# cgchemlab/chemlab

Measured on AMD Instinct MI355X. Metric: MD steps/sec, 1M-particle reactive LJ melt, higher is better.
Workload: dtype f32; 1 GPU; C5 reactive LJ melt (chain_growth_catalytic shape): 1000000 particles, rho*=0.8, rc=2.5, skin=0.3, dt=0.005, Langevin gamma=5 T=0.5, 4 reactions every 500 steps; melted for 2000 steps before the reactions start; particles=1000000, reaction_interval=500, reaction_events=2189949, parallelism=1 GPU, single domain

## Files before the change

chemlab_amd/csrc/md_kernels.hpp:

```cpp
#pragma once
#include <hip/hip_runtime.h>
#include <stdint.h>

#include "../../include/chem_mi355.h"
#include "../../include/chem_philox.h"
#include "chem_geom_host.hpp"

namespace chem {

template <typename R> struct Vec4T;
template <> struct Vec4T<float> { using type = float4; };
template <> struct Vec4T<double> { using type = double4; };
template <typename R> using Vec4 = typename Vec4T<R>::type;

template <typename R> __device__ __forceinline__ Vec4<R> mk4(R a, R b, R c, R d);
template <> __device__ __forceinline__ float4 mk4<float>(float a, float b, float c, float d) { return make_float4(a, b, c, d); }
template <> __device__ __forceinline__ double4 mk4<double>(double a, double b, double c, double d) { return make_double4(a, b, c, d); }

__device__ __forceinline__ float rint_r(float x) { return rintf(x); }
__device__ __forceinline__ double rint_r(double x) { return rint(x); }
__device__ __forceinline__ float sqrt_r(float x) { return sqrtf(x); }
__device__ __forceinline__ double sqrt_r(double x) { return sqrt(x); }
__device__ __forceinline__ float floor_r(float x) { return floorf(x); }
__device__ __forceinline__ float rcp_r(float x) { return __builtin_amdgcn_rcpf(x); }
// ... 1034 lines not shown
  __syncthreads();
}

template <typename R>
__global__ __launch_bounds__(128) void k_tile_desc(int ntiles, int CAP, const int* __restrict__ cell_start, Box<R> box,
                                                   TileLDS<R>* __restrict__ desc, DevCtl* ctl, const int* __restrict__ cell_sub) {
  if (!ctl->need_rebuild) return;
  __shared__ TileLDS<R> T;
  for (int tile = blockIdx.x; tile < ntiles; tile += gridDim.x) {
    __syncthreads();
    tile_tables<R>(T, CAP, tile, cell_start, box, ctl, cell_sub);
    const int* src = reinterpret_cast<const int*>(&T);
    int* dst = reinterpret_cast<int*>(&desc[tile]);
    for (int k = threadIdx.x; k < (int)(sizeof(TileLDS<R>) / 4); k += blockDim.x) dst[k] = src[k];
  }
}

template <typename R>
__device__ __forceinline__ void tile_load_desc(TileLDS<R>& T, const TileLDS<R>* __restrict__ desc, int tile) {
  const int* src = reinterpret_cast<const int*>(&desc[tile]);
  int* dst = reinterpret_cast<int*>(&T);
  for (int k = threadIdx.x; k < (int)(sizeof(TileLDS<R>) / 4); k += blockDim.x) dst[k] = src[k];
}

template <typename R> __device__ __forceinline__ unsigned char* d3_types(Vec4<R>* sx, int CAP) { return reinterpret_cast<unsigned char*>(sx) + (size_t)(CAP + 1) * 24; }
template <typename R, bool D3>
__device__ __forceinline__ void slot_store(Vec4<R>* const sx, const int CAP, int dst, const Vec4<R>& p) {
  if constexpr (D3) {
    R* s3 = reinterpret_cast<R*>(sx) + 3 * dst;
    s3[0] = p.x; s3[1] = p.y; s3[2] = p.z;
    d3_types<R>(sx, CAP)[dst] = (unsigned char)(int)p.w;
  } else sx[dst] = p;
}
template <typename R, int BS, bool LEAN = false, bool D3 = false, bool QW = false>
__device__ __forceinline__ void tile_fill(const TileLDS<R>& T, Vec4<R>* const sx, const int CAP,
                                          const Vec4<R>* __restrict__ x4, int wmode, const int* __restrict__ tagv = nullptr,
                                          const R* __restrict__ qtag = nullptr, R* const sq = nullptr) {
  constexpr int NW = BS / 64, RPW = (NROW + NW - 1) / NW;
  const int t = threadIdx.x;
  const int w = t >> 6, l = t & 63;
  if (t == 0) slot_store<R, D3>(sx, CAP, T.geom[3], mk4<R>((R)1e18, (R)1e18, (R)1e18, (R)0));
  if constexpr (QW) { if (t == 0) sq[T.geom[3]] = (R)0; }
  if constexpr (LEAN) {
    for (int r = w; r < NROW; r += NW) {
      const int len = T.celloff[r][SX], o0 = T.rowoff[r];
      for (int e = l; e < len; e += 64) {
        int k = 0;
#pragma unroll
        for (int q = 1; q < SX; ++q) k += (e >= T.celloff[r][q]) ? 1 : 0;
        const int g = T.cellg[r][k] + (e - T.celloff[r][k]);
        const int dst = o0 + e;
        if (dst < CAP) {
          Vec4<R> p = x4[g];
          p.x = pos_local(p.x, T.cellshx[r][k], T.org[0], T.qs[0]); p.y = pos_local(p.y, T.rowshy[r], T.org[1], T.qs[1]); p.z = pos_local(p.z, T.rowshz[r], T.org[2], T.qs[2]);
          if (wmode) p.w = idx_as_real((g << 5) | (int)p.w, (R)0);
          slot_store<R, D3>(sx, CAP, dst, p);
        }
      }
    }
    return;
  }
  Vec4<R> pv[RPW][2];
  int pk_[RPW][2], pg[RPW][2];
  [[maybe_unused]] int ptg[RPW][2];
  [[maybe_unused]] R pq[RPW][2];
#pragma unroll
  for (int rr = 0; rr < RPW; ++rr) {
    const int r = w + rr * NW;
    const int len = r < NROW ? T.celloff[r][SX] : 0;
#pragma unroll
    for (int c = 0; c < 2; ++c) {
      const int e = l + 64 * c;
      pk_[rr][c] = -1;
      if (e < len) {
        int k = 0;
#pragma unroll
        for (int q = 1; q < SX; ++q) k += (e >= T.celloff[r][q]) ? 1 : 0;
        const int g = T.cellg[r][k] + (e - T.celloff[r][k]);
        pk_[rr][c] = k; pg[rr][c] = g;
        pv[rr][c] = x4[g];
        if constexpr (QW) ptg[rr][c] = tagv[g];
      }
    }
  }
  if constexpr (QW) {
#pragma unroll
    for (int rr = 0; rr < RPW; ++rr)
#pragma unroll
      for (int c = 0; c < 2; ++c) pq[rr][c] = pk_[rr][c] >= 0 ? qtag[ptg[rr][c]] : (R)0;
  }
#pragma unroll
  for (int rr = 0; rr < RPW; ++rr) {
    const int r = w + rr * NW;
#pragma unroll
    for (int c = 0; c < 2; ++c) {
      const int k = pk_[rr][c];
      if (k >= 0) {
        const int dst = T.rowoff[r] + l + 64 * c;
        if (dst < CAP) {
          Vec4<R> p = pv[rr][c];
          p.x = pos_local(p.x, T.cellshx[r][k], T.org[0], T.qs[0]); p.y = pos_local(p.y, T.rowshy[r], T.org[1], T.qs[1]); p.z = pos_local(p.z, T.rowshz[r], T.org[2], T.qs[2]);
          if (wmode) p.w = idx_as_real((pg[rr][c] << 5) | (int)p.w, (R)0);
          slot_store<R, D3>(sx, CAP, dst, p);
          if constexpr (QW) sq[dst] = pq[rr][c];
        }
      }
    }
  }
  for (int r = w; r < NROW; r += NW) {
    const int len = T.celloff[r][SX], o0 = T.rowoff[r];
    for (int e = l + 128; e < len; e += 64) {
      int k = 0;
#pragma unroll
      for (int q = 1; q < SX; ++q) k += (e >= T.celloff[r][q]) ? 1 : 0;
      const int g = T.cellg[r][k] + (e - T.celloff[r][k]);
      const int dst = o0 + e;
      if (dst < CAP) {
        Vec4<R> p = x4[g];
        p.x = pos_local(p.x, T.cellshx[r][k], T.org[0], T.qs[0]); p.y = pos_local(p.y, T.rowshy[r], T.org[1], T.qs[1]); p.z = pos_local(p.z, T.rowshz[r], T.org[2], T.qs[2]);
        if (wmode) p.w = idx_as_real((g << 5) | (int)p.w, (R)0);
        slot_store<R, D3>(sx, CAP, dst, p);
        if constexpr (QW) sq[dst] = qtag[tagv[g]];
      }
    }
  }
}

struct ActMask { unsigned int row[kMaxTypes]; };
#define CHEM_LDS __attribute__((address_space(3)))
constexpr int NBND = SX * NSUB + 1;
#ifndef CHEM_LIST_DELTA
#define CHEM_LIST_DELTA 2.5e-4f
#endif
constexpr float kListDelta = CHEM_LIST_DELTA;
constexpr int kGrpF = 20;
struct ListLDS { int img_bytes, nwords, tmask_off, bnd_off; };
__device__ __forceinline__ ListLDS list_lds_layout(int CAP, int ntypes) {
  ListLDS L;
  L.img_bytes = (((CAP + 3) >> 2) + 3) * kGrpF * 4;
  L.nwords = ((CAP + 31) >> 5) + 2;
  L.tmask_off = L.img_bytes;
  L.bnd_off = L.tmask_off + ntypes * L.nwords * 4;
  return L;
}
__host__ __device__ constexpr size_t list_lds_bytes(int CAP, int ntypes) {
  return (size_t)(((CAP + 3) >> 2) + 3) * kGrpF * 4 + (size_t)ntypes * (((CAP + 31) >> 5) + 2) * 4 + (size_t)NROW * NBND * 2 + 16;
}

template <int BS>
__device__ __forceinline__ void list_stage_clear(unsigned char* lds, const ListLDS& L, int ntypes) {
  CHEM_LDS unsigned int* tm = (CHEM_LDS unsigned int*)((CHEM_LDS unsigned char*)lds + L.tmask_off);
  for (int k = threadIdx.x; k < ntypes * L.nwords; k += BS) tm[k] = 0u;
}
template <typename RS, int BS>
__device__ __forceinline__ void list_stage_f32(TileLDS<RS>& T, unsigned char* lds, const ListLDS& L, const int CAP,
                                               const Vec4<RS>* __restrict__ x4, const ActMask& act, int ntypes) {
  constexpr int NW = BS / 64;
  CHEM_LDS unsigned char* const l3 = (CHEM_LDS unsigned char*)lds;
  CHEM_LDS float* img = (CHEM_LDS float*)l3;
  CHEM_LDS unsigned int* tm = (CHEM_LDS unsigned int*)(l3 + L.tmask_off);
  CHEM_LDS unsigned short* bnd = (CHEM_LDS unsigned short*)(l3 + L.bnd_off);
  const int w = threadIdx.x >> 6, l = threadIdx.x & 63;
  for (int t = threadIdx.x; t < NROW * NBND; t += BS) {
    const int r = t / NBND, f = t - r * NBND, k = f >> 2, j = f & 3;
    int v = T.celloff[r][k < SX ? k : SX];
    if (k < SX && j) {
      const int pk = T.cellsub[r][k];
      if (pk < 0) { if (T.celloff[r][k + 1] > T.celloff[r][k]) T.geom[7] = 1; }
      else v += (pk >> (8 * (j - 1))) & 0xff;
    }
    bnd[t] = (unsigned short)v;
  }
  for (int r = w; r < NROW; r += NW) {
    const int len = T.celloff[r][SX], o0 = T.rowoff[r];
    for (int e0 = 0; e0 < len; e0 += 64) {
      const int e = e0 + l;
      int tj = -1;
      if (e < len) {
        int k = 0;
#pragma unroll
        for (int q = 1; q < SX; ++q) k += (e >= T.celloff[r][q]) ? 1 : 0;
        const int g = T.cellg[r][k] + (e - T.celloff[r][k]);
        const int dst = o0 + e;
        if (dst < CAP) {
          const Vec4<RS> p = x4[g];
          CHEM_LDS float* grp = img + (dst >> 2) * kGrpF + (dst & 3);
          const float u = (float)pos_local(p.x, T.cellshx[r][k], T.org[0], T.qs[0]), v = (float)pos_local(p.y, T.rowshy[r], T.org[1], T.qs[1]),
                      w_ = (float)pos_local(p.z, T.rowshz[r], T.org[2], T.qs[2]);
          grp[0] = u; grp[4] = v; grp[8] = w_; grp[12] = fmaf(u, u, fmaf(v, v, w_ * w_));
          tj = (int)p.w & 15;
        }
      }
      const int slot0 = o0 + e0, sh = slot0 & 31, wbase = slot0 >> 5;
      for (int ti = 0; ti < ntypes; ++ti) {
        const unsigned long long m = __ballot(tj >= 0 && ((act.row[ti] >> tj) & 1u));
        if (m == 0ull) continue;
        const unsigned long long lo = m << sh;
        const unsigned int w2 = sh ? (unsigned int)(m >> (64 - sh)) : 0u;
        const unsigned int part = l == 0 ? (unsigned int)lo : (l == 1 ? (unsigned int)(lo >> 32) : w2);
        if (l < 3 && part) __hip_atomic_fetch_or(&tm[ti * L.nwords + wbase + l], __brev(part), __ATOMIC_RELAXED, __HIP_MEMORY_SCOPE_WORKGROUP);
      }
    }
  }
}

typedef unsigned int u32x4_t __attribute__((ext_vector_type(4)));
__device__ __forceinline__ uint4 nt_load_u4(const uint4* p) {
  const u32x4_t v = __builtin_nontemporal_load(reinterpret_cast<const u32x4_t*>(p));
  return make_uint4(v.x, v.y, v.z, v.w);
}

__device__ __forceinline__ int xcd_remap(int bid, int nwg) {
  const int q = nwg >> 3, r = nwg & 7, xcd = bid & 7, idx = bid >> 3;
  return (xcd < r ? xcd * (q + 1) : r * (q + 1) + (xcd - r) * q) + idx;
}



template <typename R, int BS>
__device__ __forceinline__ void dev_nlist_tile(const TileLDS<R>& T, Vec4<R>* const sx, const int* tag, const R rl2,
                                               const int* excl_start, const int* excl_list, const int has_excl, const ActMask& act,
                                               unsigned short* nl16, const int S16, int* nnh, int* nlist, const int S, int* nn, DevCtl* ctl,
                                               const Box<R>* bx = nullptr, const int* rtag = nullptr, const Vec4<R>* x4 = nullptr, const R rl2_rows_ = (R)-1) {
    const R rl2_rows = rl2_rows_ > (R)0 ? rl2_rows_ : rl2;
    const int hx = T.geom[0], total = T.geom[3], nhome = T.geom[4], hbase = T.geom[5];
    unsigned short* reg16 = nl16 + (size_t)hbase * S16;
    for (int q = threadIdx.x; q < nhome; q += BS) {
      int sgi = 0;
#pragma unroll
      for (int k = 1; k < NHSEG; ++k) sgi += (q >= T.hoff[k]) ? 1 : 0;
      const int inrun = q - T.hoff[sgi];
      const int p = T.hstart[sgi] + inrun;
      const int ly = sgi % HY, lz = sgi / HY;
      const int hr = (lz + 1) * SY + (ly + 1);
      const int eh = inrun + T.celloff[hr][1];
      int lx = 0;
      for (int k = 2; k <= hx; ++k) lx += (eh >= T.celloff[hr][k]) ? 1 : 0;
      const int sself = T.rowoff[hr] + eh;
      const Vec4<R> xi = sx[sself];
      const unsigned int arow = act.row[real_as_idx(xi.w) & 15];
      int e0 = 0, e1 = 0;
      if (has_excl) { const int tg = tag[p]; e0 = excl_start[tg]; e1 = excl_start[tg + 1]; }
      int cnt = 0, cnt16 = 0;
      int* row32 = nlist ? nlist + (size_t)p * S : nullptr;
      uint4* regq = reinterpret_cast<uint4*>(reg16) + q;
      uint4 acc = make_uint4(0, 0, 0, 0);
      auto push = [&](unsigned int sl) {
        acc.x = __builtin_amdgcn_alignbit(acc.y, acc.x, 16);
        acc.y = __builtin_amdgcn_alignbit(acc.z, acc.y, 16);
        acc.z = __builtin_amdgcn_alignbit(acc.w, acc.z, 16);
        acc.w = (acc.w >> 16) | (sl << 16);
        if ((cnt16 & 7) == 7 && cnt16 < S16) regq[(size_t)(cnt16 >> 3) * nhome] = acc;
        ++cnt16;
      };
      auto hit = [&](int s, int jw) {
        const int j = jw >> 5;
        bool ok = j != p;
        if (ok && e1 > e0) {
          const int tgj = tag[j];
          for (int e = e0; e < e1; ++e) if (excl_list[e] == tgj) { ok = false; break; }
        }
        if (ok) {
          if ((arow >> (jw & 15)) & 1u) push((unsigned int)s);
          if (row32) {
            bool in_rows = true;
            if (rl2_rows < rl2) { const Vec4<R> xj = sx[s]; const R dx = xi.x - xj.x, dy_ = xi.y - xj.y, dz_ = xi.z - xj.z; in_rows = dx * dx + dy_ * dy_ + dz_ * dz_ <= rl2_rows; }
            if (in_rows) { if (cnt < S) row32[cnt] = j; ++cnt; }
          }
        }
      };
      auto suboff = [&](int r, int f, bool lower) {
        const int k = f >> 2, j = f & 3;
        const int base = T.celloff[r][k];
        if (j == 0) return base;
        const int pk = T.cellsub[r][k];
        if (pk < 0) return lower ? base : T.celloff[r][k + 1];
        return base + ((pk >> (8 * (j - 1))) & 0xff);
      };
#pragma unroll 1
      for (int dzy = 0; dzy < 9; ++dzy) {
        const int dz = dzy / 3, dy = dzy - 3 * dz;
        const int r = (lz + dz) * SY + (ly + dy);
        const R weps = T.clen[0] * (R)2e-4;
        const R ylo = ((R)(ly + 1) - (R)kRefCells) * T.clen[1], zlo = ((R)(lz + 1) - (R)kRefCells) * T.clen[2];
        R ddy = dy == 0 ? xi.y - ylo - weps : (dy == 2 ? ylo + T.clen[1] - xi.y - weps : (R)0);
        R ddz = dz == 0 ? xi.z - zlo - weps : (dz == 2 ? zlo + T.clen[2] - xi.z - weps : (R)0);
        ddy = ddy > 0 ? ddy : (R)0; ddz = ddz > 0 ? ddz : (R)0;
        const R w2 = rl2 - ddy * ddy - ddz * ddz;
        if (w2 < (R)0) continue;
        const R ws = (sqrt_r(w2) + weps) * T.subinv, sxi = (xi.x + (R)kRefCells * T.clen[0]) * T.subinv;
        int f_lo = (int)(sxi - ws), f_hi = (int)(sxi + ws);
        f_lo = f_lo > lx * NSUB ? f_lo : lx * NSUB;
        f_hi = f_hi < (lx + 3) * NSUB - 1 ? f_hi : (lx + 3) * NSUB - 1;
        const int a = T.rowoff[r] + suboff(r, f_lo, true);
        int b = T.rowoff[r] + suboff(r, f_hi + 1, false);
        b = b < total ? b : total;
        for (int s0 = a; s0 < b; s0 += 64) {
          const int len = (b - s0) < 64 ? (b - s0) : 64;
          unsigned int mlo = 0, mhi = 0;
          for (int k = 0; k < len; k += 4) {
            Vec4<R> xj[4];
#pragma unroll
            for (int u = 0; u < 4; ++u) xj[u] = sx[(k + u < len) ? s0 + k + u : total];
            unsigned int bits = 0;
#pragma unroll
            for (int u = 0; u < 4; ++u) {
              const R dx = xi.x - xj[u].x, dy_ = xi.y - xj[u].y, dz_ = xi.z - xj[u].z;
              const R r2 = dx * dx + dy_ * dy_ + dz_ * dz_;
              bits |= (r2 <= rl2) ? (1u << u) : 0u;
            }
            if (k < 32) mlo |= bits << k; else mhi |= bits << (k - 32);
          }
          unsigned long long m = ((unsigned long long)mhi << 32) | mlo;
          while (m) {
            const int k = __ffsll((long long)m) - 1;
            m &= m - 1;
            const int s = s0 + k;
            hit(s, real_as_idx(sx[s].w));
          }
        }
      }
      const int real16 = cnt16;
      if (real16 <= S16) while (cnt16 & 7) push((unsigned int)total);
      nnh[hbase + q] = real16 < S16 ? real16 : S16;
      if (real16 > S16) atomicMax(&ctl->nl_overflow, real16);
      if (row32) {
        const int c32 = cnt < S ? cnt : S;
        for (int k = c32; k < ((c32 + 3) & ~3); ++k) row32[k] = p;
        nn[p] = c32;
        if (cnt > S) atomicMax(&ctl->nl_overflow, cnt);
      }
    }
}

template <typename RS, int BS>
__device__ __forceinline__ void dev_nlist_tile_f32(const TileLDS<RS>& T, unsigned char* lds, const ListLDS& L, const int* tag, const float rl2,
                                                   const int* excl_start, const int* excl_list, const int has_excl,
                                                   unsigned short* nl16, const int S16, int* nnh, int* nlist, const int S, int* nn, DevCtl* ctl,
                                                   const Box<RS>* bx, const int* rtag, const Vec4<RS>* x4, const int ablate = 0, const float rl2_rows_ = -1.f,
                                                   uint4* bslots = nullptr, const int* gtag = nullptr, const int real0 = 0, const int real1 = 0x7fffffff,
                                                   const int coop_on = 0) {
  const float rl2_rows = rl2_rows_ > 0.f ? rl2_rows_ : rl2;
  typedef float f32x4 __attribute__((ext_vector_type(4)));
  typedef float f32x2 __attribute__((ext_vector_type(2)));
  typedef __attribute__((address_space(3))) const volatile f32x4 lds_f32x4;
  CHEM_LDS unsigned char* const l3 = (CHEM_LDS unsigned char*)lds;
  const CHEM_LDS float* img = (const CHEM_LDS float*)l3;
  const CHEM_LDS unsigned int* tmask = (const CHEM_LDS unsigned int*)(l3 + L.tmask_off);
  const CHEM_LDS unsigned short* bnd = (const CHEM_LDS unsigned short*)(l3 + L.bnd_off);
  const int hx = T.geom[0], total = T.geom[3], nhome = T.geom[4], hbase = T.geom[5];
  const bool nowin = T.geom[7] != 0;
  unsigned short* reg16 = nl16 + (size_t)hbase * S16;
  const float clen0 = (float)T.clen[0], clen1 = (float)T.clen[1], clen2 = (float)T.clen[2], subinv = (float)T.subinv;
// ... 1042 lines not shown
};

__device__ __forceinline__ bool grid_barrier(GridBar* gb, DevCtl* ctl) {
  __shared__ int ok_s;
  asm volatile("s_waitcnt vmcnt(0)" ::: "memory");
  __syncthreads();
  if (threadIdx.x == 0) {
    __builtin_amdgcn_fence(__ATOMIC_RELEASE, "agent");
    int ok = 1;
    const unsigned int g = blockIdx.x & 7u;
    const unsigned int ngrp = gridDim.x < 8u ? gridDim.x : 8u;
    const unsigned int gsize = (gridDim.x - g + 7u) >> 3;
    const unsigned int gen = __hip_atomic_load(&gb->gen[0], __ATOMIC_RELAXED, __HIP_MEMORY_SCOPE_AGENT);
    if (atomicAdd(&gb->grp[g][0], 1u) == gsize - 1u) {
      __hip_atomic_store(&gb->grp[g][0], 0u, __ATOMIC_RELAXED, __HIP_MEMORY_SCOPE_AGENT);
      if (atomicAdd(&gb->top[0], 1u) == ngrp - 1u) {
        __hip_atomic_store(&gb->top[0], 0u, __ATOMIC_RELAXED, __HIP_MEMORY_SCOPE_AGENT);
        __hip_atomic_fetch_add(&gb->gen[0], 1u, __ATOMIC_RELEASE, __HIP_MEMORY_SCOPE_AGENT);
      }
    }
    unsigned int spins = 0;
    while (__hip_atomic_load(&gb->gen[0], __ATOMIC_RELAXED, __HIP_MEMORY_SCOPE_AGENT) == gen) {
      __builtin_amdgcn_s_sleep(8);
      if (++spins > (1u << 20)) { ctl->barrier_timeout = 1; ok = 0; break; }
    }
    __builtin_amdgcn_fence(__ATOMIC_ACQUIRE, "agent");
    ok_s = ok;
  }
  __syncthreads();
  return ok_s != 0;
}

template <typename R> struct FusedArgs {
  int n, ncell, ntiles, CAP, S, has_excl, criterion, par, seg_shift, tseg_shift, nblk, want32, ntypes, ablate, coop;
  double half_skin; R rl2;
  long long istep;
  double half_skin_ref; R rl2_rows;
  Vec4<R> *x4, *v4, *x4o, *v4o, *x0;
  int *tag, *tago, *rtag; int4 *img4, *img4o;
  int *cell_cnt, *cell_of, *slot_of, *cell_start, *cell_loc, *btot, *perm, *tn, *tloc, *tbtot, *cell_sub, *cell_n, *bucket; int bcap;
  TileLDS<R>* desc; const int *excl_start, *excl_list;
  int* tile_ord;
  int* tile_pos;
  unsigned short* nl16; int *nnh, *nlist, *nn;
  unsigned long long* blockmax; DevCtl* ctl; GridBar* gb;
  const int* bstart; const BondedEntry* bent; int4 *bwork, *bj; int nbent;
  uint4* bslots;
  int bond_pass;
  Box<R> box; ActMask act;
  long long* wgst;
};

template <int BS>
__device__ __forceinline__ void seg_offsets(const int* tot, int nseg, int* s_off) {
  int carry = 0;
  for (int base = 0; base < nseg; base += BS) {
    const int k = base + (int)threadIdx.x;
    const int v = k < nseg ? tot[k] : 0;
    int t;
    const int ex = block_scan_excl<BS>(v, &t);
    if (k < nseg) s_off[k] = carry + ex;
    carry += t;
  }
  if (threadIdx.x == 0) s_off[nseg] = carry;
  __syncthreads();
}

template <int BS>
__device__ __forceinline__ void seg_scan(int* cnt, int nitem, int shift, int* loc, int* tot, bool zero, int* cnt_copy = nullptr) {
  const int per = 1 << shift, nseg = (nitem + per - 1) >> shift;
  for (int seg = blockIdx.x; seg < nseg; seg += gridDim.x) {
    const int lo = seg << shift, hi = min(nitem, lo + per);
    int carry = 0;
    for (int base = lo; base < hi; base += BS) {
      const int k = base + (int)threadIdx.x;
      int v = 0;
      if (k < hi) { v = cnt[k]; if (zero) cnt[k] = 0; if (cnt_copy) cnt_copy[k] = v; }
      int t;
      const int ex = block_scan_excl<BS>(v, &t);
      if (k < hi) loc[k] = carry + ex;
      carry += t;
    }
    if (threadIdx.x == 0) tot[seg] = carry;
  }
}

#ifndef CHEM_FUSED_WAVES
#define CHEM_FUSED_WAVES 4
#endif
template <typename R, int BS, bool DIAG = false>
__global__ __launch_bounds__(BS, CHEM_FUSED_WAVES) void k_rebuild_fused(const FusedArgs<R> a) {
  __shared__ TileLDS<R> T;
  __shared__ int s_off[1025];
  __shared__ unsigned long long s_m[BS / 64];
  __shared__ int s_tile;
  CHEM_DYN_LDS(R);
  const int t = threadIdx.x, b = blockIdx.x, NB = gridDim.x, lane = lane_id(), w = t >> 6;
  DevCtl* const ctl = a.ctl;

  if (ctl->halt) return;
  unsigned long long m = 0;
  for (int k = t; k < a.nblk; k += BS) { const unsigned long long v = a.blockmax[k]; m = v > m ? v : m; }
  for (int o = 32; o > 0; o >>= 1) { const unsigned long long v = __shfl_xor(m, o); m = v > m ? v : m; }
  if (lane == 0) s_m[w] = m;
  __syncthreads();
  m = s_m[0];
#pragma unroll
  for (int k = 1; k < BS / 64; ++k) m = s_m[k] > m ? s_m[k] : m;
  const double m2 = sizeof(R) == 4 ? bits_real_f(m) : bits_real_d(m);
  double acc = a.criterion ? sqrt(m2) : ctl->acc_pp[a.par] + sqrt(m2);
  const int forced = ctl->force_rebuild;
  const int need = (acc > a.half_skin) || forced;
  auto ref_update = [&]() {
    const double accr = a.criterion ? sqrt(m2) : ctl->acc_ref + sqrt(m2);
    const bool rn = (accr > a.half_skin_ref) || forced;
    ctl->acc_ref = rn ? 0.0 : accr;
    if (rn) ctl->ref_rebuilds++;
  };
  if (!need) {
    if (b == 0 && t == 0) { ctl->step_m2 = m2; ctl->acc_pp[a.par ^ 1] = acc; ctl->acc_maxdist = acc; ctl->need_rebuild = 0; ref_update(); }
    return;
  }

  if (b == 0 && t == 0) a.gb->stamp[0] = wall_clock64();
  long long* const wst = (DIAG && a.wgst) ? a.wgst + 8 * (size_t)b : nullptr;
  const int ablate = DIAG ? a.ablate : 0;
#define WGST(K) do { if (wst && t == 0) wst[K] = wall_clock64(); } while (0)
  WGST(0);
  if (b == 0 && t < 8) a.gb->tq[t][0] = 0u;
  if (b == 0 && t == 8) { ctl->bw64 = 0ull; a.gb->prepq[0] = 0u; }
  { MigBuf<R> none{}; dev_bin<R>(0, a.n, a.x4, a.v4, a.tag, a.img4, a.box, a.cell_cnt, a.cell_of, a.slot_of, none, none, ctl, a.bucket, a.bcap, a.btot, a.seg_shift); }
  WGST(1);
  if (!grid_barrier(a.gb, ctl)) return; WGST(2); if (b == 0 && t == 0) { const long long st = wall_clock64(); a.gb->stamp[1] = st; a.gb->stamp[2] = st; a.gb->stamp[3] = st; }
  if (ctl->bucket_overflow) {
    for (int k = b * BS + t; k < a.ncell; k += NB * BS) a.cell_cnt[k] = 0;
    if (b == 0) for (int k = t; k < 1024; k += BS) a.btot[k] = 0;
    if (b == 0 && t == 0) { ctl->need_rebuild = 1; ctl->force_rebuild = 1; ctl->halt_step = a.istep; ctl->halt = 1; }
    return;
  }
  if (b == 0 && t == 0) {
    ctl->step_m2 = m2; ctl->acc_pp[a.par ^ 1] = 0.0; ctl->acc_maxdist = 0.0; ctl->force_rebuild = 0;
    ctl->rebuild_count++; ctl->need_rebuild = 1;
    ref_update();
  }

  {
    const int nseg = (a.ncell + (1 << a.seg_shift) - 1) >> a.seg_shift;
    seg_offsets<BS>(a.btot, nseg, s_off);
    if (b == 0 && t == 0) a.cell_start[a.ncell] = s_off[nseg];
    dev_sort_gather_bucket<R>(a.ncell, a.cell_cnt, s_off, a.seg_shift, a.bucket, a.bcap, a.cell_start, a.x4, a.v4, a.tag, a.img4,
                              a.x4o, a.v4o, a.tago, a.img4o, a.rtag, a.box, a.cell_sub);
    const int nx = a.box.nc[0], ny = a.box.nc[1], nz = a.box.nc[2];
    const int ntx = tile_ntx(nx, a.box.xs_nb, a.box.xs_w), nty = (ny + HY - 1) / HY;
    for (int tile = b * BS + t; tile < a.ntiles; tile += NB * BS) {
      const int tx = tile % ntx, ty = (tile / ntx) % nty, tz = tile / (ntx * nty);
      int cx0, hx;
      tile_xrange(tx, nx, a.box.xs_nb, a.box.xs_w, cx0, hx);
      const int cy0 = ty * HY, cz0 = tz * HZ;
      const int hy = min(HY, ny - cy0), hz = min(HZ, nz - cz0);
      int nh = 0;
      for (int hzi = 0; hzi < hz; ++hzi) for (int hyi = 0; hyi < hy; ++hyi) {
        const int c0 = ((cz0 + hzi) * ny + (cy0 + hyi)) * nx + cx0;
        for (int k = 0; k < hx; ++k) nh += a.cell_cnt[c0 + k];
      }
      a.tn[tile] = nh;
    }
  }
  WGST(3);
  if (!grid_barrier(a.gb, ctl)) return; WGST(4); if (b == 0 && t == 0) { const long long st = wall_clock64(); a.gb->stamp[4] = st; a.gb->stamp[5] = st; }

  {
    for (int k = b * BS + t; k < a.ncell; k += NB * BS) a.cell_cnt[k] = 0;
    if (b == 0) for (int k = t; k < 1024; k += BS) a.btot[k] = 0;
    const int tper = 1 << a.tseg_shift, ntseg = (a.ntiles + tper - 1) >> a.tseg_shift;
    {
      int carry = 0;
      for (int base = 0; base < ntseg; base += BS) {
        const int k = base + t;
        int v = 0;
        if (k < ntseg) for (int j = k << a.tseg_shift; j < min(a.ntiles, (k + 1) << a.tseg_shift); ++j) v += a.tn[j];
        int tot;
        const int ex = block_scan_excl<BS>(v, &tot);
        if (k < ntseg) s_off[k] = carry + ex;
        carry += tot;
      }
      __syncthreads();
    }
    const int q = a.ntiles >> 3, r = a.ntiles & 7, myx = b & 7;
    const int lpar = a.tile_ord ? (ctl->rebuild_count & 1) : 0;
    const int* const ord_r = a.tile_ord ? a.tile_ord + (size_t)lpar * a.ntiles : nullptr;
    const int* const pos_r = a.tile_pos ? a.tile_pos + (size_t)lpar * a.ntiles : nullptr;
    int ndone = 0;
    WGST(5);
    auto claim = [&]() {
      int tile = -1;
      for (int d = 0; d < 8 && tile < 0; ++d) {
        const int x = (myx + d) & 7;
        const int cntx = q + (x < r ? 1 : 0);
        if (__hip_atomic_load(&a.gb->tq[x][0], __ATOMIC_RELAXED, __HIP_MEMORY_SCOPE_AGENT) >= (unsigned int)cntx) continue;
        const int k = (int)atomicAdd(&a.gb->tq[x][0], 1u);
        if (k < cntx) { tile = (x < r ? x * (q + 1) : r * (q + 1) + (x - r) * q) + k; if (ord_r) tile = ord_r[tile]; }
      }
      return tile;
    };
    for (;;) {
      __syncthreads();
      if (t == 0) s_tile = claim();
      __syncthreads();
      const int tile = s_tile;
      if (tile < 0) break;
      ++ndone;
      int hb_part = 0;
      if (w == BS / 64 - 1) {
        for (int j = ((tile >> a.tseg_shift) << a.tseg_shift) + lane; j < tile; j += 64) hb_part += a.tn[j];
      }
      const bool f32list = sizeof(R) == 4 || !(DIAG && a.want32);
      if (f32list) list_stage_clear<BS>(chem_dyn_lds, list_lds_layout(a.CAP, a.ntypes), a.ntypes);
      tile_tables<R>(T, a.CAP, tile, a.cell_start, a.box, ctl, a.cell_sub);
      if (w == BS / 64 - 1) {
        for (int o = 32; o > 0; o >>= 1) hb_part += __shfl_xor(hb_part, o);
        if (lane == 0) T.geom[5] = s_off[tile >> a.tseg_shift] + hb_part;
      }
      __syncthreads();
      {
        const int* src = reinterpret_cast<const int*>(&T);
        int* dst = reinterpret_cast<int*>(&a.desc[pos_r ? pos_r[tile] : tile]);
        for (int k = t; k < (int)(sizeof(TileLDS<R>) / 4); k += BS) dst[k] = src[k];
      }
      if (f32list) {
        const ListLDS L = list_lds_layout(a.CAP, a.ntypes);
        list_stage_f32<R, BS>(T, chem_dyn_lds, L, a.CAP, a.x4o, a.act, a.ntypes);
        __syncthreads();
        if (ablate == 1) { for (int q = t; q < T.geom[4]; q += BS) a.nnh[T.geom[5] + q] = 0; }
        else
        dev_nlist_tile_f32<R, BS>(T, chem_dyn_lds, L, a.tago, (float)a.rl2, a.excl_start, a.excl_list, a.bond_pass ? 0 : a.has_excl, a.nl16, a.S, a.nnh,
                               (DIAG && a.want32) ? a.nlist : (int*)nullptr, a.S, a.nn, ctl, &a.box, a.rtag, a.x4o, ablate, (float)a.rl2_rows,
                               a.bond_pass ? (uint4*)nullptr : a.bslots, nullptr, 0, 0x7fffffff, a.coop);
      } else {
        tile_fill<R, BS, true>(T, sx, a.CAP, a.x4o, 1);
        __syncthreads();
        dev_nlist_tile<R, BS>(T, sx, a.tago, a.rl2, a.excl_start, a.excl_list, a.has_excl, a.act, a.nl16, a.S, a.nnh,
                              a.want32 ? a.nlist : (int*)nullptr, a.S, a.nn, ctl, &a.box, a.rtag, a.x4o, a.rl2_rows);
      }
    }
    WGST(6);
    if (wst && t == 0) wst[7] = ndone;
    if (a.tile_ord && b < 8 && w == 0) {
      const int cntx = q + (b < r ? 1 : 0), off = b < r ? b * (q + 1) : r * (q + 1) + (b - r) * q;
      int* const ord_w = a.tile_ord + (size_t)(lpar ^ 1) * a.ntiles;
      int* const pos_w = a.tile_pos + (size_t)(lpar ^ 1) * a.ntiles;
      const int mean4 = (int)(((long long)a.n * 4 + a.ntiles - 1) / a.ntiles);
      auto cls_of = [&](int tile) { const int c = a.tn[tile] * 16 / (mean4 > 0 ? mean4 : 1); return 7 - (c > 7 ? 7 : c); };
      int tot[8] = {0, 0, 0, 0, 0, 0, 0, 0};
      for (int k0 = 0; k0 < cntx; k0 += 64) {
        const int k = k0 + lane, c = k < cntx ? cls_of(off + k) : -1;
#pragma unroll
        for (int cc = 0; cc < 8; ++cc) tot[cc] += __popcll(__ballot(c == cc));
      }
      int base[8]; { int acc_ = 0;
#pragma unroll
        for (int cc = 0; cc < 8; ++cc) { base[cc] = acc_; acc_ += tot[cc]; } }
      for (int k0 = 0; k0 < cntx; k0 += 64) {
        const int k = k0 + lane, c = k < cntx ? cls_of(off + k) : -1;
#pragma unroll
        for (int cc = 0; cc < 8; ++cc) {
          const unsigned long long m = __ballot(c == cc);
          if (c == cc) { const int p_ = off + base[cc] + __popcll(m & lanemask_lt()); ord_w[p_] = off + k; pos_w[off + k] = p_; }
          base[cc] += __popcll(m);
        }
      }
    }
    if (a.nbent > 0) {
      for (;;) {
        __syncthreads();
        if (t == 0) s_tile = (int)atomicAdd(&a.gb->prepq[0], 1u);
        __syncthreads();
        const int ib = s_tile * BS;
        if (ib >= a.n) break;
        dev_bonded_prep_chunk<BS>(ib, a.n, a.tago, a.rtag, a.bstart, a.bent, a.bwork, a.bj, ctl, a.bslots ? a.excl_start : (const int*)nullptr);
      }
    }
    for (int k = b * BS + t; k < a.n; k += NB * BS) {
      const Vec4<R> xk = a.x4o[k];
      a.x4[k] = xk; if (a.x0) a.x0[k] = xk;
      a.v4[k] = a.v4o[k]; a.img4[k] = a.img4o[k]; a.tag[k] = a.tago[k];
    }
  }
  if (t == 0) {
    const volatile DevCtl* vc = ctl;
    if (vc->stage_overflow | vc->nl_overflow) { ctl->halt_step = a.istep; ctl->halt = 1; }
  }
  if (b == 0 && t == 0) a.gb->stamp[6] = wall_clock64();
  if (wst) { __syncthreads(); if (t == 0) wst[7] |= (long long)(wall_clock64() - wst[0]) << 16; }
#undef WGST
}

template <typename R>
__global__ __launch_bounds__(256) void k_kinetic(int i0, int n, const Vec4<R>* __restrict__ v4, double* __restrict__ out) {
  const int i = i0 + blockIdx.x * blockDim.x + threadIdx.x;
  double ek = 0, px = 0, py = 0, pz = 0;
  if (i < i0 + n) {
    const Vec4<R> v = v4[i];
    const double m = (double)v.w, vx = (double)v.x, vy = (double)v.y, vz = (double)v.z;
    ek = 0.5 * m * (vx * vx + vy * vy + vz * vz); px = m * vx; py = m * vy; pz = m * vz;
  }
  __shared__ double red[4][4];
  for (int o = 32; o > 0; o >>= 1) { ek += __shfl_xor(ek, o); px += __shfl_xor(px, o); py += __shfl_xor(py, o); pz += __shfl_xor(pz, o); }
  if (lane_id() == 0) { int w = threadIdx.x >> 6; red[0][w] = ek; red[1][w] = px; red[2][w] = py; red[3][w] = pz; }
  __syncthreads();
  if (threadIdx.x < 4) {
    double s = 0;
    for (int k = 0; k < (int)(blockDim.x >> 6); ++k) s += red[threadIdx.x][k];
    out[4 * blockIdx.x + threadIdx.x] = s;
  }
}

__global__ __launch_bounds__(256) void k_rescale_lambda(const double* __restrict__ part, int nblk, double* __restrict__ ekin_io, double* __restrict__ lam_out,
                                                        int kind, double kT, double pref , double ntot, uint64_t svr_seed, uint64_t step) {
  __shared__ double red[4];
  double ek = 0;
  for (int k = threadIdx.x; k < nblk; k += blockDim.x) ek += part[4 * k];
  for (int o = 32; o > 0; o >>= 1) ek += __shfl_xor(ek, o);
  if (lane_id() == 0) red[threadIdx.x >> 6] = ek;
  __syncthreads();
  if (threadIdx.x == 0) {
    if (nblk > 0) { ek = red[0] + red[1] + red[2] + red[3]; *ekin_io = ek; }
    else ek = *ekin_io;
    if (lam_out) {
      const double kTnow = 2.0 * ek / (3.0 * ntot);
      *lam_out = kind == 1 ? sqrt(1.0 + pref * (kT / kTnow - 1.0)) : kind == 2 ? sqrt(kT / kTnow)
               : chem_philox::svr_lambda(svr_seed, step, ek, 1.5 * ntot * kT, (int64_t)(3.0 * ntot), 1.0 / pref);
    }
  }
}
template <typename R>
__global__ __launch_bounds__(256) void k_scale_v(int i0, int n, Vec4<R>* __restrict__ v4, const double* __restrict__ lam, const DevCtl* __restrict__ ctl) {
  if (ctl->halt) return;
  const int i = i0 + blockIdx.x * blockDim.x + threadIdx.x;
  if (i >= i0 + n) return;
  const R s = (R)*lam;
  Vec4<R> v = v4[i];
  v.x *= s; v.y *= s; v.z *= s;
  v4[i] = v;
}

struct ReactionDev {
  int type_1, type_2, delta_1, delta_2;
  int min1, max1, min2, max2;
  int intramolecular, intraresidual, active, restricted;
  int cons_role, pad_;
  double cut2, mincut2, prob;
};
struct ReactSet { int n; uint64_t seed; uint64_t step; int nearest; ReactionDev r[CHEM_MAX_REACTIONS]; };
struct ConnTable { const int* start; const int* partner; const unsigned int* mask; const unsigned int* cons_ok; };
__device__ __forceinline__ bool conn_allows(const ConnTable& ct, int ta, int tb, int q) {
  if (!ct.start) return false;
  for (int e = ct.start[ta]; e < ct.start[ta + 1]; ++e) if (ct.partner[e] == tb) return (ct.mask[e] >> q) & 1u;
  return false;
}

struct Candidate { int a, b, r; unsigned int h; double d2; };

template <typename R>
__global__ __launch_bounds__(256) void k_react_scan(int i0, int n, const Vec4<R>* __restrict__ x4, const int* __restrict__ tag,
                                                    const int* __restrict__ nlist, const int* __restrict__ nn, int S,
                                                    const int* __restrict__ state, const int* __restrict__ res_id,
                                                    const int* __restrict__ mol_id, BoxD box, const ReactSet* __restrict__ rs_g,
                                                    Candidate* __restrict__ cand, int cand_cap, DevCtl* ctl, ConnTable conn) {
  __shared__ ReactSet rs;
  {
    const int* src = reinterpret_cast<const int*>(rs_g);
    int* dst = reinterpret_cast<int*>(&rs);
    for (int k = threadIdx.x; k < (int)(sizeof(ReactSet) / 4); k += blockDim.x) dst[k] = src[k];
  }
  __syncthreads();
  constexpr int TPP = 8;
  constexpr int kWaveBuf = 192;
  __shared__ Candidate sbuf[4 * kWaveBuf];
  Candidate* wbuf = sbuf + (threadIdx.x >> 6) * kWaveBuf;
  int wcount = 0;
  const int gid = blockIdx.x * blockDim.x + threadIdx.x;
  const int i = i0 + gid / TPP, sub = gid % TPP;
  int cnt = 0, ti = 0, si = 0, tgi = 0, ri = 0, mi = 0;
  Vec4<R> xi = mk4<R>(0, 0, 0, 0);
  const int* row = nullptr;
  if (i < i0 + n) {
    xi = x4[i]; ti = (int)xi.w; tgi = tag[i]; si = state[tgi]; ri = res_id[tgi]; mi = mol_id[tgi];
    cnt = nn[i]; row = nlist + (size_t)i * S;
    bool any = false;
    for (int q = 0; q < rs.n; ++q) {
      const ReactionDev& R_ = rs.r[q];
// ... 590 lines not shown
```

Baseline: 7430 steps/s.

## Restructure neighbor-list staging as flat slot sweep with prefetched loads overlapping descriptor write

The per-tile list staging now walks all slots of the tile flatly across the whole block instead of per-row per-wave. It issues up to NF position loads per thread into registers before doing the descriptor finish, barrier and bound-table work, so global latency overlaps that setup. Because each wave now covers 32-aligned slots, the type-mask atomics become plain stores. Per-tile home counts are also computed one wave per tile with one lane per cell and a shuffle reduction, instead of one thread looping serially. The trade-offs are more register pressure from the prefetch arrays and a geom[7] flag that is now written as zero into the global descriptor.

```diff
diff --git a/chemlab_amd/csrc/md_kernels.hpp b/chemlab_amd/csrc/md_kernels.hpp
--- a/chemlab_amd/csrc/md_kernels.hpp
+++ b/chemlab_amd/csrc/md_kernels.hpp
@@ -1210,53 +1210,75 @@
   CHEM_LDS unsigned int* tm = (CHEM_LDS unsigned int*)((CHEM_LDS unsigned char*)lds + L.tmask_off);
   for (int k = threadIdx.x; k < ntypes * L.nwords; k += BS) tm[k] = 0u;
 }
-template <typename RS, int BS>
+struct StageNoMid { __device__ __forceinline__ void operator()() const {} };
+template <typename RS, int BS, typename Mid = StageNoMid>
 __device__ __forceinline__ void list_stage_f32(TileLDS<RS>& T, unsigned char* lds, const ListLDS& L, const int CAP,
-                                               const Vec4<RS>* __restrict__ x4, const ActMask& act, int ntypes) {
-  constexpr int NW = BS / 64;
+                                               const Vec4<RS>* __restrict__ x4, const ActMask& act, int ntypes, Mid&& mid = Mid()) {
+  static_assert(BS % 64 == 0 && NROW <= 64, "a wave stages 64 consecutive slots; one lane per row offset");
+  constexpr int NF = sizeof(RS) == 8 ? 3 : 6;
   CHEM_LDS unsigned char* const l3 = (CHEM_LDS unsigned char*)lds;
   CHEM_LDS float* img = (CHEM_LDS float*)l3;
   CHEM_LDS unsigned int* tm = (CHEM_LDS unsigned int*)(l3 + L.tmask_off);
   CHEM_LDS unsigned short* bnd = (CHEM_LDS unsigned short*)(l3 + L.bnd_off);
-  const int w = threadIdx.x >> 6, l = threadIdx.x & 63;
-  for (int t = threadIdx.x; t < NROW * NBND; t += BS) {
-    const int r = t / NBND, f = t - r * NBND, k = f >> 2, j = f & 3;
-    int v = T.celloff[r][k < SX ? k : SX];
-    if (k < SX && j) {
-      const int pk = T.cellsub[r][k];
-      if (pk < 0) { if (T.celloff[r][k + 1] > T.celloff[r][k]) T.geom[7] = 1; }
-      else v += (pk >> (8 * (j - 1))) & 0xff;
-    }
-    bnd[t] = (unsigned short)v;
-  }
-  for (int r = w; r < NROW; r += NW) {
-    const int len = T.celloff[r][SX], o0 = T.rowoff[r];
-    for (int e0 = 0; e0 < len; e0 += 64) {
-      const int e = e0 + l;
-      int tj = -1;
-      if (e < len) {
+  const int l = threadIdx.x & 63;
+  const int total = T.rowoff[NROW], lim = total < CAP ? total : CAP;
+  const int ro_l = T.rowoff[l < NROW ? l : NROW];
+  int ro[NROW];
+#pragma unroll
+  for (int q = 1; q < NROW; ++q) ro[q] = __builtin_amdgcn_readlane(ro_l, q);
+  for (int s0 = 0; s0 < lim; s0 += NF * BS) {
+    Vec4<RS> pv[NF];
+    int prk[NF];
+#pragma unroll
+    for (int c = 0; c < NF; ++c) {
+      const int s = s0 + c * BS + (int)threadIdx.x;
+      prk[c] = -1;
+      if (s < lim) {
+        int r = 0, o0 = 0;
+#pragma unroll
+        for (int q = 1; q < NROW; ++q) if (s >= ro[q]) { r = q; o0 = ro[q]; }
+        const int e = s - o0;
         int k = 0;
 #pragma unroll
         for (int q = 1; q < SX; ++q) k += (e >= T.celloff[r][q]) ? 1 : 0;
         const int g = T.cellg[r][k] + (e - T.celloff[r][k]);
-        const int dst = o0 + e;
-        if (dst < CAP) {
-          const Vec4<RS> p = x4[g];
-          CHEM_LDS float* grp = img + (dst >> 2) * kGrpF + (dst & 3);
-          const float u = (float)pos_local(p.x, T.cellshx[r][k], T.org[0], T.qs[0]), v = (float)pos_local(p.y, T.rowshy[r], T.org[1], T.qs[1]),
-                      w_ = (float)pos_local(p.z, T.rowshz[r], T.org[2], T.qs[2]);
-          grp[0] = u; grp[4] = v; grp[8] = w_; grp[12] = fmaf(u, u, fmaf(v, v, w_ * w_));
-          tj = (int)p.w & 15;
+        prk[c] = (r << 3) | k;
+        pv[c] = x4[g];
+      }
+    }
+    if (s0 == 0) {
+      mid();
+      for (int t = threadIdx.x; t < NROW * NBND; t += BS) {
+        const int r = t / NBND, f = t - r * NBND, k = f >> 2, j = f & 3;
+        int v = T.celloff[r][k < SX ? k : SX];
+        if (k < SX && j) {
+          const int pk = T.cellsub[r][k];
+          if (pk < 0) { if (T.celloff[r][k + 1] > T.celloff[r][k]) T.geom[7] = 1; }
+          else v += (pk >> (8 * (j - 1))) & 0xff;
         }
-      }
-      const int slot0 = o0 + e0, sh = slot0 & 31, wbase = slot0 >> 5;
+        bnd[t] = (unsigned short)v;
+      }
+    }
+#pragma unroll
+    for (int c = 0; c < NF; ++c) {
+      const int slot0 = s0 + c * BS + ((int)threadIdx.x & ~63);
+      if (slot0 >= lim) continue;
+      int tj = -1;
+      if (prk[c] >= 0) {
+        const int r = prk[c] >> 3, k = prk[c] & 7, dst = slot0 + l;
+        const Vec4<RS> p = pv[c];
+        CHEM_LDS float* grp = img + (dst >> 2) * kGrpF + (dst & 3);
+        const float u = (float)pos_local(p.x, T.cellshx[r][k], T.org[0], T.qs[0]), v = (float)pos_local(p.y, T.rowshy[r], T.org[1], T.qs[1]),
+                    w_ = (float)pos_local(p.z, T.rowshz[r], T.org[2], T.qs[2]);
+        grp[0] = u; grp[4] = v; grp[8] = w_; grp[12] = fmaf(u, u, fmaf(v, v, w_ * w_));
+        tj = (int)p.w & 15;
+      }
+      const int wbase = slot0 >> 5;
       for (int ti = 0; ti < ntypes; ++ti) {
         const unsigned long long m = __ballot(tj >= 0 && ((act.row[ti] >> tj) & 1u));
         if (m == 0ull) continue;
-        const unsigned long long lo = m << sh;
-        const unsigned int w2 = sh ? (unsigned int)(m >> (64 - sh)) : 0u;
-        const unsigned int part = l == 0 ? (unsigned int)lo : (l == 1 ? (unsigned int)(lo >> 32) : w2);
-        if (l < 3 && part) __hip_atomic_fetch_or(&tm[ti * L.nwords + wbase + l], __brev(part), __ATOMIC_RELAXED, __HIP_MEMORY_SCOPE_WORKGROUP);
+        const unsigned int part = l == 0 ? (unsigned int)m : (unsigned int)(m >> 32);
+        if (l < 2 && part) tm[ti * L.nwords + wbase + l] = __brev(part);
       }
     }
   }
@@ -2605,18 +2627,17 @@
                               a.x4o, a.v4o, a.tago, a.img4o, a.rtag, a.box, a.cell_sub);
     const int nx = a.box.nc[0], ny = a.box.nc[1], nz = a.box.nc[2];
     const int ntx = tile_ntx(nx, a.box.xs_nb, a.box.xs_w), nty = (ny + HY - 1) / HY;
-    for (int tile = b * BS + t; tile < a.ntiles; tile += NB * BS) {
+    static_assert(HX * HY * HZ <= 64, "one lane per home cell");
+    for (int tile = b * (BS / 64) + w; tile < a.ntiles; tile += NB * (BS / 64)) {
       const int tx = tile % ntx, ty = (tile / ntx) % nty, tz = tile / (ntx * nty);
       int cx0, hx;
       tile_xrange(tx, nx, a.box.xs_nb, a.box.xs_w, cx0, hx);
       const int cy0 = ty * HY, cz0 = tz * HZ;
       const int hy = min(HY, ny - cy0), hz = min(HZ, nz - cz0);
-      int nh = 0;
-      for (int hzi = 0; hzi < hz; ++hzi) for (int hyi = 0; hyi < hy; ++hyi) {
-        const int c0 = ((cz0 + hzi) * ny + (cy0 + hyi)) * nx + cx0;
-        for (int k = 0; k < hx; ++k) nh += a.cell_cnt[c0 + k];
-      }
-      a.tn[tile] = nh;
+      const int k = lane % HX, hyi = (lane / HX) % HY, hzi = lane / (HX * HY);
+      int nh = (k < hx && hyi < hy && hzi < hz) ? a.cell_cnt[((cz0 + hzi) * ny + (cy0 + hyi)) * nx + cx0 + k] : 0;
+      for (int o = 32; o > 0; o >>= 1) nh += __shfl_xor(nh, o);
+      if (lane == 0) a.tn[tile] = nh;
     }
   }
   WGST(3);
@@ -2670,19 +2691,20 @@
       const bool f32list = sizeof(R) == 4 || !(DIAG && a.want32);
       if (f32list) list_stage_clear<BS>(chem_dyn_lds, list_lds_layout(a.CAP, a.ntypes), a.ntypes);
       tile_tables<R>(T, a.CAP, tile, a.cell_start, a.box, ctl, a.cell_sub);
-      if (w == BS / 64 - 1) {
-        for (int o = 32; o > 0; o >>= 1) hb_part += __shfl_xor(hb_part, o);
-        if (lane == 0) T.geom[5] = s_off[tile >> a.tseg_shift] + hb_part;
-      }
-      __syncthreads();
-      {
+      auto finish_desc = [&]() __attribute__((always_inline)) {
+        if (w == BS / 64 - 1) {
+          for (int o = 32; o > 0; o >>= 1) hb_part += __shfl_xor(hb_part, o);
+          if (lane == 0) T.geom[5] = s_off[tile >> a.tseg_shift] + hb_part;
+        }
+        __syncthreads();
         const int* src = reinterpret_cast<const int*>(&T);
         int* dst = reinterpret_cast<int*>(&a.desc[pos_r ? pos_r[tile] : tile]);
-        for (int k = t; k < (int)(sizeof(TileLDS<R>) / 4); k += BS) dst[k] = src[k];
-      }
+        constexpr int kG7 = (int)(offsetof(TileLDS<R>, geom) / 4) + 7;
+        for (int k = t; k < (int)(sizeof(TileLDS<R>) / 4); k += BS) dst[k] = k == kG7 ? 0 : src[k];
+      };
       if (f32list) {
         const ListLDS L = list_lds_layout(a.CAP, a.ntypes);
-        list_stage_f32<R, BS>(T, chem_dyn_lds, L, a.CAP, a.x4o, a.act, a.ntypes);
+        list_stage_f32<R, BS>(T, chem_dyn_lds, L, a.CAP, a.x4o, a.act, a.ntypes, finish_desc);
         __syncthreads();
         if (ablate == 1) { for (int q = t; q < T.geom[4]; q += BS) a.nnh[T.geom[5] + q] = 0; }
         else
@@ -2690,6 +2712,7 @@
                                (DIAG && a.want32) ? a.nlist : (int*)nullptr, a.S, a.nn, ctl, &a.box, a.rtag, a.x4o, ablate, (float)a.rl2_rows,
                                a.bond_pass ? (uint4*)nullptr : a.bslots, nullptr, 0, 0x7fffffff, a.coop);
       } else {
+        finish_desc();
         tile_fill<R, BS, true>(T, sx, a.CAP, a.x4o, 1);
         __syncthreads();
         dev_nlist_tile<R, BS>(T, sx, a.tago, a.rl2, a.excl_start, a.excl_list, a.has_excl, a.act, a.nl16, a.S, a.nnh,
```

Result: no change. 7399 steps/s (-0.4%).
